# snu-mllab/Q-Palette

Hardware: AMD Instinct MI355X
Metric: decode tokens/s bs=1 Llama-3.1-8B @3.25b; achieved HBM GB/s vs peak (higher is better)
Workload: dtype f16 weights x f16 activations, f32 accumulate

## Files before the change

### include/qpal.h

```cpp
#ifndef QPAL_H
#define QPAL_H

#include <stdint.h>

#ifdef __cplusplus
extern "C" {
#endif

#define QPAL_VERSION 300

#define QPAL_OK 0
#define QPAL_E_SHAPE (-1)
#define QPAL_E_PARAM (-2)
#define QPAL_E_NULL (-3)
#define QPAL_E_ALIGN (-4)

#define QPAL_SPLIT_NONE 0
#define QPAL_SPLIT_ROWS 1
#define QPAL_SPLIT_COLS 2

int qpal_tcq_gemv(float *out, const void *c1, const void *c2, const void *x, const void *tlut,
                  int m, int n, int k, int S, int KV1, int KV2, int split, void *stream);

typedef struct qpal_tcq_job {
// ... 162 lines not shown

int qpal_lm_head_logits(const float *h_f32, long ld_h, const void *rms_w_f16, float rms_eps, const void *w_f16, float *logits_f32,
                        long ld_logits, int rows, int vocab, int k, void *stream);

int qpal_sample(const float *logits_f32, long ld_logits, int rows, int vocab, const float *temperature, const int *top_k,
                const float *top_p, const long *seed, const long *ctr, long *token, void *stream);

int qpal_token_logprob(const float *logits_f32, long ld_logits, int rows, int vocab, const long long *token, float *logprob,
                       float *lse, int *rank, const long long *active, void *stream);

int qpal_spec_draft(const int *hist, long ld_hist, const long *n_tok, const long *limit, const long *ext_draft, const int *ext_n,
                    int B, int K, int gmin, int gmax, int R, long max_len, long *tokens, int *seq, int *row0, long *pos0,
                    int *row_slot, long *row_ctr, int *n_draft, void *stream);
int qpal_spec_accept(const long *tokens, const long *drawn, const int *seq, const int *row0, int *hist, long ld_hist, long *n_tok,
                     long *limit, const long *eos, int B, int K, int R, long *out_tok, int *n_out, int *n_acc, void *stream);

int qpal_logit_process(const float *logits_f32, long ld_logits, float *out_f32, long ld_out, int rows, int vocab, const int *row_slot,
                       const long *ctr, int slots, const int *count, long ld_count, const float *repetition, const float *presence,
                       const float *frequency, const unsigned *mask, long ld_mask, const int *mask_on, const int *bias_id,
                       const float *bias_val, const int *bias_n, int bias_slots, const long *tokens, const int *row0, void *stream);
int qpal_logit_observe(int *count, long ld_count, int slots, int vocab, const int *slot, int slot0, const long *tokens,
                       const long *active, int n, void *stream);

#define QPAL_HESSIAN_TILE 128
int qpal_hessian_accum(double *H, double *colsum, const void *X_f16, long ld_x, int rows, int n, void *stream);

int qpal_lora_apply(float *out_f32, long ld_out, const void *in, int in_mode, float rms_eps, const void *rms_weight, const void *A,
                    const void *B, const int *blk_off, const int *blk_m, int P, const int *row_adapter, int rows, int k, int R, int N,
                    void *stream);

int qpal_plan_gemv(const int *rows, const int *steps1, const int *steps2, const int *flags, int njobs, int waves, int shared_staging,
                   int *out, int out_len);

int qpal_can_fuse_rotation(int n, int k);
int qpal_can_fuse_rotation_k(int n, int k, int K);

int qpal_calib_stream_read(const void *const *srcs, const long *bytes, int nseg, void *sink, int grid, void *stream);
int qpal_calib_decode_rate(const void *tlut, void *sink, int iters, int S, int KV, int grid, void *stream);

const char *qpal_error_string(int code);
int qpal_version(void);

#ifdef __cplusplus
}
#endif
#endif
```

### q-palette_amd/_native.py

```python
import ctypes
import os
import subprocess

_HERE = os.path.dirname(os.path.abspath(__file__))
SO_PATH = os.environ.get("QPAL_LIB") or os.path.join(_HERE, "libqpal_hip.so")
_lib = None

QPAL_SPLIT_NONE, QPAL_SPLIT_ROWS, QPAL_SPLIT_COLS = 0, 1, 2

_P, _I, _F = ctypes.c_void_p, ctypes.c_int, ctypes.c_float


class TcqJob(ctypes.Structure):
    _fields_ = [("out", _P), ("c1", _P), ("c2", _P), ("x", _P), ("tlut", _P), ("m", _I), ("k", _I),
                ("out_zeroed", _I), ("wscale", _P), ("oscale", _F), ("ldo", ctypes.c_long),
                ("x_had", _I), ("x_post", _F), ("x_su", _P), ("kv", _I),
                ("x_f32", _P),
                ("x_rms_eps", _F), ("x_rms_w", _P), ("accumulate", _I), ("kv2", _I), ("act_out", _P), ("x_hadk", _P), ("x_K", _I), ("act_su", _P)]


class LutJob(ctypes.Structure):
    _fields_ = [("out", _P), ("qweight", _P), ("x", _P), ("lut", _P), ("m", _I), ("k", _I), ("out_zeroed", _I),
                ("wscale", _P), ("oscale", _F), ("ldo", ctypes.c_long), ("x_had", _I), ("x_post", _F), ("x_su", _P),
                ("x_f32", _P),
                ("x_rms_eps", _F), ("x_rms_w", _P), ("accumulate", _I), ("act_out", _P), ("x_hadk", _P), ("x_K", _I), ("act_su", _P)]


PEER_WS_BYTES_PER_SLOT = 256
IPC_HANDLE_BYTES = 64


_SIGNATURES = {
    "qpal_tcq_gemv_multi": [ctypes.POINTER(TcqJob), _I, _I, _I, _I, _I, _I, _P, ctypes.c_long, _P],
    "qpal_lut_tc_gemv_multi": [ctypes.POINTER(LutJob), _I, _I, _I, _I, _P, ctypes.c_long, _P],
    "qpal_tcq_gemv": [_P, _P, _P, _P, _P, _I, _I, _I, _I, _I, _I, _I, _P],
    "qpal_tcq_dequant": [_P, _P, _P, _P, _I, _I, _I, _I, _I, _I, _P],
    "qpal_lut_tc_gemv": [_P, _P, _P, _P, _I, _I, _I, _I, _I, _P],
    "qpal_lut_tc_dequant": [_P, _P, _P, _I, _I, _I, _I, _P],
    "qpal_lut_simt_gemv": [_P, _P, _P, _P, _I, _I, _I, _I, _I, _P],
    "qpal_lut_simt_dequant": [_P, _P, _P, _I, _I, _I, _I, _P],
    "qpal_tc_to_simt": [_P, _P, _I, _I, _I, _I, _P],
    "qpal_plan_gemv": [ctypes.POINTER(_I), ctypes.POINTER(_I), ctypes.POINTER(_I), ctypes.POINTER(_I), _I, _I, _I, ctypes.POINTER(_I), _I],
    "qpal_can_fuse_rotation": [_I, _I],
    "qpal_can_fuse_rotation_k": [_I, _I, _I],
    "qpal_pack_tcq": [_P, _P, _I, _I, _I],
    "qpal_pack_tcq_states": [_P, _P, _I, _I, _I],
    "qpal_pack_lut_tc": [_P, _P, _I, _I, _I, _I],
    "qpal_pack_lut_simt": [_P, _P, _I, _I, _I, _I],
    "qpal_hadamard": [_P, _P, _P, _P, _P, _I, _I, _I, _I, _I, _I, _F, _P],
    "qpal_hadamard_rms": [_P, _P, _P, _F, _P, _P, _I, _I, _I, _F, _P],
    "qpal_hadamard_f32": [_P, _P, _P, _P, _I, _I, _I, _I, _F, _P],
    "qpal_rope_kv": [_P, _P, _P, _P, _P, _P, _P, _P, _I, _I, _I, ctypes.c_long, _P],
    "qpal_attn_decode": [_P, _P, _P, _P, _P, _I, _I, _I, ctypes.c_long, _F, _P],
    "qpal_attn_rope_decode": [_P, _P, _P, _P, _P, _P, _P, _P, _I, _I, _I, ctypes.c_long, _F, _P, ctypes.c_long, _P],
    "qpal_attn_ws_bytes": [_I, _I, _I, ctypes.c_long],
    "qpal_attn_rope_decode_batch": [_P, _P, _P, ctypes.c_long, _P, _P, _P, ctypes.c_long, _P, _P, _I, _I, _I, _I, ctypes.c_long, _F,
                                    _P, ctypes.c_long, _P],
    "qpal_attn_batch_ws_bytes": [_I, _I, _I, _I, ctypes.c_long],
    "qpal_attn_rope_prefill": [_P, _P, _P, ctypes.c_long, _P, _P, _P, ctypes.c_long, _P, _P, _I, _I, _I, _I, ctypes.c_long, _F,
                               _P, ctypes.c_long, _P],
    "qpal_attn_prefill_ws_bytes": [_I, _I, _I, _I, ctypes.c_long],
    "qpal_attn_rope_decode_batch_kv8": [_P, _P, _P, ctypes.c_long, _P, _P, _P, ctypes.c_long, _P, _P, _I, _I, _I, _I, ctypes.c_long,
                                        _F, _P, ctypes.c_long, _P],
    "qpal_attn_rope_prefill_kv8": [_P, _P, _P, ctypes.c_long, _P, _P, _P, ctypes.c_long, _P, _P, _I, _I, _I, _I, ctypes.c_long, _F,
                                   _P, ctypes.c_long, _P],
    "qpal_attn_rope_decode_batch_paged": [_P, _P, _P, ctypes.c_long, _P, _P, _P, ctypes.c_long, _P, _P, _P, ctypes.c_long, _I, _I, _I, _I,
                                          _I, _I, _I, _I, _F, _P, ctypes.c_long, _P],
    "qpal_attn_rope_prefill_paged": [_P, _P, _P, ctypes.c_long, _P, _P, _P, ctypes.c_long, _P, _P, _P, _I, _I, _I, _I,
                                     _I, _I, _I, _I, _F, _P, ctypes.c_long, _P],
    "qpal_attn_ragged_ws_bytes": [_I, _I, _I, _I, _I, ctypes.c_long],
    "qpal_attn_rope_prefill_ragged": [_P, _P, _P, ctypes.c_long, _P, _P, _P, ctypes.c_long, _P, _P, _P, _P, _I, _I, _I, _I, _I, _I, _I,
                                      ctypes.c_long, _F, _P, ctypes.c_long, _P],
    "qpal_attn_rope_prefill_ragged_paged": [_P, _P, _P, ctypes.c_long, _P, _P, _P, ctypes.c_long, _P, _P, _P, _P, _P, ctypes.c_long, _I,
                                            _I, _I, _I, _I, _I, _I, _I, _I, _I, _F, _P, ctypes.c_long, _P],
    "qpal_lm_head_argmax": [_P, _P, _F, _P, _P, _P, _P, ctypes.c_long, _I, _I, _P],
# ... 73 lines not shown
```

### q-palette_amd/csrc/qpal_capi.hip

```cpp
#include <stdio.h>
#include <hip/hip_runtime.h>
#include <math.h>
#include <stdlib.h>

#include "lut_kernels_api.h"
#include "tcq_kernels_api.h"
#include "tc_gemm16.h"
#include <string.h>

using namespace qpal;

namespace {

constexpr int kMaxBatch = 128;

int nbg_of(int n) { return n <= 8 ? 1 : n <= 16 ? 2 : n <= 32 ? 4 : n <= 64 ? 8 : n <= 80 ? 10 : 16; }
int waves_of(int nbg) { return gemv_waves<1>() == 8 ? 8 : (nbg >= 4 ? 8 : 16); }
int round_capacity(int waves) {
#if defined(QPAL_W8) && !defined(QPAL_W8_ONE)
    return waves == 8 ? 2 * kNumCU : kNumCU;
#else
    (void)waves;
    return kNumCU;
#endif
// ... 49 lines not shown
        if (!x_hadk || !p.x) return QPAL_E_NULL;
        if (x_f32 || x_rms_eps > 0.f) return QPAL_E_PARAM;
        if (!aligned(p.x, 16) || (x_su && !aligned(x_su, 16)) || !aligned(x_hadk, 2)) return QPAL_E_ALIGN;
        p.x_rot = kK28;
        p.x_hadk = static_cast<const uint16_t *>(x_hadk);
        p.x_su = static_cast<const uint16_t *>(x_su);
        p.x_pre = (float)(1.0 / sqrt((double)k));
        p.x_post = x_post;
        return QPAL_OK;
    }
    if (!rot_ok(n, k)) return QPAL_E_SHAPE;
    if (x_su && !aligned(x_su, 16)) return QPAL_E_ALIGN;
    if (x_f32) {
        p.x = static_cast<const uint16_t *>(x_f32);
        p.x_src_f32 = 1;
    }
    if (!p.x) return QPAL_E_NULL;
    if (x_rms_w && !aligned(x_rms_w, 16)) return QPAL_E_ALIGN;
    p.x_rms_eps = x_rms_eps > 0.f ? x_rms_eps : 0.f;
    p.x_rms_w = static_cast<const uint16_t *>(x_rms_w);
    if (!aligned(p.x, 16)) return QPAL_E_ALIGN;
    p.x_rot = k / 1024;
    p.x_su = static_cast<const uint16_t *>(x_su);
    p.x_pre = (float)(1.0 / sqrt((double)k));
    p.x_post = x_post;
    return QPAL_OK;
}

int nb_of(int n) { return n <= 1 ? 1 : n <= 2 ? 2 : n <= 4 ? 4 : 8; }

static int env_int(const char *name, int dflt) {
    const char *v = getenv(name);
    return v ? atoi(v) : dflt;
}

struct TapePlan {
    LaunchPlan lp;
    int cost;
    bool shared;
    bool ok;
};

TapePlan tape_plan(int lg_g, int rg, int st1, int st2, int W) {
    TapePlan tp{};
    const int G = 1 << lg_g, st = st1 + st2;
    tp.lp.lg_g = lg_g;
    tp.lp.rg = rg;
    const long T = (long)rg * st;
    if (st <= 0 || rg < 1 || rg > 255 || T < G) return tp;
    struct Piece { int row, stream, s0, len; };
    for (int m = 0; m < G; m++) {
        const long t0 = T * m / G, t1 = T * (m + 1) / G;
        Piece pc[kPlanWaves];
        int np = 0;
        for (int r = (int)(t0 / st); r < rg && (long)r * st < t1; r++)
            for (int sidx = 0; sidx < 2; sidx++) {
                const long seg0 = (long)r * st + (sidx ? st1 : 0), seg1 = seg0 + (sidx ? st2 : st1);
                const long a = seg0 > t0 ? seg0 : t0, b = seg1 < t1 ? seg1 : t1;
                if (b <= a) continue;
                if (np == W) return tp;
                pc[np++] = Piece{r, sidx, (int)(a - seg0), (int)(b - a)};
            }
        const long L = t1 - t0;
        struct Slot { int piece, part, ns; };
        Slot best_slots[kPlanWaves];
        int best_nslots = 0, best_cost = 1 << 30, best_long = 1 << 30;
// ... 6 lines not shown
                per[i] = pc[i].len / nw[i];
                if (per[i] < rowmin[pc[i].row]) rowmin[pc[i].row] = per[i];
            }
            for (int i = 1; i < np; i++)
                for (int k = i; k > 0; k--) {
                    const int x = order[k - 1], y = order[k];
                    const bool swap = rowmin[pc[y].row] != rowmin[pc[x].row] ? rowmin[pc[y].row] > rowmin[pc[x].row]
                                      : pc[y].row != pc[x].row             ? pc[y].row < pc[x].row
                                                                           : per[y] > per[x];
                    if (!swap) break;
                    order[k - 1] = y;
                    order[k] = x;
                }
            Slot slots[kPlanWaves];
            int simd[4] = {0, 0, 0, 0}, w = 0, longest = 0;
            for (int oi = 0; oi < np; oi++) {
                const int i = order[oi];
                for (int part = 0; part < nw[i]; part++, w++) {
                    const int ns = pc[i].len / nw[i] + (part < pc[i].len % nw[i] ? 1 : 0);
                    slots[w] = Slot{i, part, ns};
                    simd[w & 3] += ns;
                    if (ns > longest) longest = ns;
                }
            }
            int c = simd[0];
            for (int sd = 1; sd < 4; sd++) c = simd[sd] > c ? simd[sd] : c;
            if (c < best_cost || (c == best_cost && longest < best_long)) {
                best_cost = c;
                best_long = longest;
                best_nslots = w;
                for (int k = 0; k < w; k++) best_slots[k] = slots[k];
            }
        };
        for (int q = q0 > 0 ? q0 : 1; q <= 4 * q0 + 4; q++) {
            int nw[kPlanWaves], used = 0;
            for (int i = 0; i < np; i++) {
                nw[i] = (pc[i].len + q - 1) / q;
                used += nw[i];
            }
            if (used > W) continue;
            consider(nw);
            const int spare = W - used;
            if (spare == 0) continue;
            {
                int g[kPlanWaves];
                for (int i = 0; i < np; i++) g[i] = nw[i];
                for (int k = 0; k < spare; k++) {
                    int at = -1, worst = 0;
                    for (int i = 0; i < np; i++) {
                        const int pr = (pc[i].len + g[i] - 1) / g[i];
                        if (g[i] < pc[i].len && pr > worst) { worst = pr; at = i; }
                    }
                    if (at < 0) break;
                    g[at]++;
                }
                consider(g);
            }
            for (int t = 0; t < np; t++) {
                int g[kPlanWaves];
                for (int i = 0; i < np; i++) g[i] = nw[i];
                g[t] = g[t] + spare < pc[t].len ? g[t] + spare : pc[t].len;
                consider(g);
            }
        }
        if (best_cost == 1 << 30) return tp;
        int wave = best_nslots;
        for (int k = 0; k < best_nslots; k++) {
            const Piece &pp = pc[best_slots[k].piece];
            int nparts = 0;
            for (int k2 = 0; k2 < best_nslots; k2++) nparts += best_slots[k2].piece == best_slots[k].piece;
            const int base = pp.len / nparts, rem = pp.len % nparts, part = best_slots[k].part;
            const int s0 = pp.s0 + part * base + (part < rem ? part : rem);
            if (best_slots[k].ns > 0xffff || s0 > 0xffff) return tp;
            WaveEnt &e = tp.lp.w[m][k];
            e.a = (uint32_t)pp.row | ((uint32_t)pp.stream << 8) | (1u << 16);
            e.b = (uint32_t)s0 | ((uint32_t)best_slots[k].ns << 16);
// ... 8 lines not shown
        for (int sd = 0; sd < 4; sd++) {
            int c = 0;
            for (int q = 0; q < per; q++) c += (int)(tp.lp.w[m][sd + 4 * q].b >> 16);
            if (c > tp.cost) tp.cost = c;
        }
    }
    for (int r = 0; r < rg; r++) {
        int owners = 0;
        for (int m = 0; m < G; m++) {
            bool has = false;
            for (int w = 0; w < W; w++) has = has || ((tp.lp.w[m][w].a >> 16 & 1u) && (int)(tp.lp.w[m][w].a & 255u) == r);
            owners += has;
        }
        if (owners > 2) return tp;
        if (owners > 1) {
            tp.shared = true;
            for (int m = 0; m < G; m++)
                for (int w = 0; w < W; w++)
                    if ((tp.lp.w[m][w].a >> 16 & 1u) && (int)(tp.lp.w[m][w].a & 255u) == r) tp.lp.w[m][w].a |= 1u << 10;
        }
    }
    tp.ok = true;
    return tp;
}

int class_rows(const TcMultiParams &mp, int c, int rg) {
    int rows = 0;
    for (int j = 0; j < mp.njobs; j++)
        if (mp.job[j].cls == c) rows += (mp.job[j].nrows + rg - 1) / rg * rg;
    return rows;
}

void plan_launch(TcMultiParams &mp, const int *out_zeroed, int &grid, int waves = 16) {
    static const int force_g = env_int("QPAL_FORCE_G", 0);
    static const int force_rg = env_int("QPAL_FORCE_RG", 0);
    static const int share_on = env_int("QPAL_SHARE", env_int("QPAL_PAIR", 1));
    const int cap = round_capacity(waves);
    int ncls = 0, cst1[2] = {0, 0}, cst2[2] = {0, 0};
    for (int j = 0; j < mp.njobs; j++) {
        TcParams &p = mp.job[j];
        int c = 0;
        while (c < ncls && (cst1[c] != p.st1 || cst2[c] != p.st2)) c++;
        if (c == ncls) {
            if (ncls == 2) c = 1;
            else { cst1[c] = p.st1; cst2[c] = p.st2; ncls++; }
        }
        p.cls = c;
    }
    bool free_share = share_on != 0, swiglu = false;
    for (int j = 0; j < mp.njobs; j++) {
        const TcParams &p = mp.job[j];
        if (!((out_zeroed && out_zeroed[j]) || p.accumulate)) free_share = false;
        swiglu = swiglu || p.act_out != nullptr;
    }
    constexpr int kMemsetCost = 10;
    constexpr int kRoundCost = 4;
    struct Cand { TapePlan tp; int lg_g, rg; };
    static thread_local Cand cands[2][3 * 64];
    int ncand[2] = {0, 0};
    for (int c = 0; c < ncls; c++)
        for (int lg = 0; lg <= 2; lg++) {
            if (force_g > 0 && (1 << lg) != force_g) continue;
            if (swiglu && lg != 0) continue;
            for (int rg = 1; rg <= 16 << lg && rg <= 64; rg++) {
                if (force_rg > 0 && rg != force_rg) continue;
                if (swiglu && (rg & (rg - 1) || rg < 2 || rg > waves)) continue;
                TapePlan tp = tape_plan(lg, rg, cst1[c], cst2[c], waves);
                if (!tp.ok) continue;
                if (tp.shared && swiglu) continue;
                cands[c][ncand[c]++] = Cand{tp, lg, rg};
// ... 609 lines not shown
    if (grid > kNumCU) grid = kNumCU;
    return launch_simt_dequant(p, bits, vec, grid, static_cast<hipStream_t>(stream));
}

int qpal_tc_to_simt(void *dst_simt, const void *src_tc, int m, int k, int bits, int vec, void *stream) {
    if (!dst_simt || !src_tc) return QPAL_E_NULL;
    if (m <= 0 || k <= 0 || m % 32 || k % 32 || k % (32 * vec)) return QPAL_E_SHAPE;
    if (!(vec == 1 || vec == 2) || !lut_tc_ok(bits, vec) || ((long)bits * k) % (32 * vec)) return QPAL_E_PARAM;
    if (!aligned(dst_simt, 4) || !aligned(src_tc, 4)) return QPAL_E_ALIGN;
    hipStream_t s = static_cast<hipStream_t>(stream);
    hipError_t e = hipMemsetAsync(dst_simt, 0, (size_t)m * k / vec * bits / 8, s);
    if (e != hipSuccess) return (int)e;
    return launch_tc_to_simt(static_cast<uint32_t *>(dst_simt), static_cast<const uint32_t *>(src_tc), m, k, bits, vec, s);
}

int qpal_plan_gemv(const int *rows, const int *steps1, const int *steps2, const int *flags, int njobs, int waves, int shared_staging,
                   int *out, int out_len) {
    if (!rows || !steps1 || !steps2 || !flags || !out) return QPAL_E_NULL;
    if (njobs < 1 || njobs > kMaxJobs || (waves != 16 && waves != 8)) return QPAL_E_SHAPE;
    TcMultiParams mp{};
    mp.njobs = njobs;
    int zeroed[kMaxJobs] = {0};
    static const uint16_t dummy_x[8] = {0};
    for (int j = 0; j < njobs; j++) {
        TcParams &p = mp.job[j];
        p.nrows = rows[j];
        p.st1 = steps1[j];
        p.st2 = steps2[j];
        p.nsc1 = steps1[j] * 4;
        p.nsc2 = steps2[j] * 4;
        p.n = 1;
        p.k = (steps1[j] + steps2[j]) * 128;
        p.x = dummy_x;
        (void)shared_staging;
        zeroed[j] = flags[j] & 1;
        p.accumulate = (flags[j] >> 1) & 1;
        p.act_out = (flags[j] >> 2) & 1 ? reinterpret_cast<uint16_t *>(8) : nullptr;
        if (rows[j] < 1 || steps1[j] < 1 || steps2[j] < 0) return QPAL_E_SHAPE;
    }
    if (!gemv_classes_ok(mp)) return QPAL_E_PARAM;
    int grid = 0;
    plan_launch(mp, zeroed, grid, waves);
    const int need = 8 + 2 * (2 + 2 * kPlanMembers * kPlanWaves) + 4 * njobs;
    if (out_len < need) return QPAL_E_SHAPE;
    int o = 0;
    out[o++] = grid;
    out[o++] = mp.total_items;
    out[o++] = mp.ncls;
    out[o++] = mp.items0;
    out[o++] = 0;
    out[o++] = mp.cls_mask;
    out[o++] = kPlanMembers;
    out[o++] = kPlanWaves;
    for (int c = 0; c < 2; c++) {
        out[o++] = mp.plan[c].lg_g;
        out[o++] = mp.plan[c].rg;
        for (int m = 0; m < kPlanMembers; m++)
            for (int w = 0; w < kPlanWaves; w++) {
                out[o++] = (int)mp.plan[c].w[m][w].a;
                out[o++] = (int)mp.plan[c].w[m][w].b;
            }
    }
    for (int j = 0; j < njobs; j++) {
        out[o++] = mp.job[j].cls;
        out[o++] = mp.job[j].vrow0;
        out[o++] = mp.row_end[j];
        out[o++] = mp.job[j].sk;
    }
    return QPAL_OK;
}

int qpal_can_fuse_rotation(int n, int k) { return n >= 1 && k > 0 && rot_ok(n, k) ? 1 : 0; }
int qpal_can_fuse_rotation_k(int n, int k, int K) {
    if (K <= 1) return qpal_can_fuse_rotation(n, k);
    return rot_k28_ok(n, k, K, 64 * 1024) ? 1 : 0;
}

const char *qpal_error_string(int code) {
    switch (code) {
        case QPAL_OK: return "ok";
        case QPAL_E_SHAPE: return "unsupported shape (need m%32==0, k%32==0, 1<=n<=128; see include/qpal.h)";
        case QPAL_E_PARAM: return "unsupported quantizer parameters (S/KV/bits/vec/split)";
        case QPAL_E_NULL: return "null pointer";
        case QPAL_E_ALIGN: return "misaligned pointer";
        default: return code > 0 ? hipGetErrorString(static_cast<hipError_t>(code)) : "unknown qpal error";
    }
}

int qpal_version(void) { return QPAL_VERSION; }

}
```

### q-palette_amd/csrc/tc_kernels.h

```cpp
#pragma once
#include "qpal_common.h"
#include "wht64.h"
#include "rot_k28.h"

namespace qpal {

struct TcParams {
    float *out;
    uint16_t *wout;
    long ldo;
    long ldw;
    const uint32_t *c1;
    const uint32_t *c2;
    const uint16_t *x;
    const void *tab;
    int n;
    int k;
    int nrows;
    int nsc1, nsc2;
    int st1, st2;
    int col2;
    int sk;
    int nitems;
    int x_lds;
// ... 488 lines not shown
        xz = reinterpret_cast<const char *>(xs) + zero_off * 2;
        dead = (sv.nsc - (lane >> 4) + 3) >> 2;
        if (QPAL_ZERO_B != 0 && (c >> 1) >= n) dead = 0;
    }
    auto step_x = [&](int s, u32x4(&xb)[NBG][2]) {
        if constexpr (XLDS == 2 && NBG == 1) {
            const char *row = s < dead ? xl + s * 256 : xz;
            xb[0][0] = *reinterpret_cast<const u32x4 *>(row);
            xb[0][1] = *reinterpret_cast<const u32x4 *>(row + 16);
        } else {
            load_step_x<XLDS, NBG>(sv, xg, xs, k, n, zero_off, s, lane, xb);
        }
    };
    for (int s = s0; s < s1; s += 2) {
        {
            const int sn = s + 1 < s1 ? s + 1 : s;
            load_step_w_buf<Codec::NW>(rs, sn, lane, wb);
            __builtin_amdgcn_sched_barrier(0);
            u32x4 xb[NBG][2];
            step_x(s, xb);
            gemv_step_any<Codec, NBG>(lut, laneoff, w, xb, acc);
        }
        if (s + 1 < s1) {
            const int sn = s + 2 < s1 ? s + 2 : s + 1;
            load_step_w_buf<Codec::NW>(rs, sn, lane, w);
            __builtin_amdgcn_sched_barrier(0);
            u32x4 xb[NBG][2];
            step_x(s + 1, xb);
            gemv_step_any<Codec, NBG>(lut, laneoff, wb, xb, acc);
        }
    }
}

#ifdef QPAL_W8
template <int NBG>
constexpr int gemv_waves() { return 8; }
#define QPAL_GEMV_BOUNDS(NBG) __launch_bounds__(512, (NBG) <= 2 ? 4 : 2)
#else
template <int NBG>
constexpr int gemv_waves() { return NBG >= 4 ? 8 : 16; }
#define QPAL_GEMV_BOUNDS(NBG) __launch_bounds__(64 * gemv_waves<NBG>())
#endif
template <int NBG>
constexpr int scratch_bytes() { return NBG == 1 ? kScratchBytes : gemv_waves<NBG>() * 32 * 4 * 8 * NBG; }

template <int S>
struct TcqAny : TcqCodec<S, (S == 9 ? 8 : 10)> {
    static constexpr bool kAny = true;
    static constexpr int kMinKV = S == 9 ? 2 : S == 10 ? 8 : 9;
    static constexpr int kMaxKV = S == 9 ? 8 : 10;
};
template <class C>
constexpr bool is_any_v = requires { C::kAny; };

template <int S, class F>
__device__ __forceinline__ void dispatch_kv(int kv, F &&f) {
    static_for<TcqAny<S>::kMinKV, TcqAny<S>::kMaxKV + 1>([&](auto kc) {
        if (kv == decltype(kc)::value) f(kc);
    });
}

#ifdef QPAL_W8
constexpr int kEarlyXChunks = 1;
#else
constexpr int kEarlyXChunks = 2;
#endif
// ... 4 lines not shown
    int on;
    const uint16_t *su;
    const uint16_t *rw;
    float pre, post;
    int ie;
};

inline TcEarly early_args(const TcMultiParams &mp, int grid) {
    const TcParams &a = mp.job[0];
    TcEarly e{a.x, a.tab, a.n, a.k, a.x_lds && !a.x_rot && a.n <= 8 && a.n * a.k + 32 <= kEarlyXChunks * 64 * gemv_waves<1>() * 8 ? 1 : 0,
              a.x_su, a.x_rms_w, a.x_pre, a.x_post};
    if (a.x_lds && a.x_rot == kK28 && a.n == 1 && a.x_hadk && !a.x_src_f32 && !(a.x_rms_eps > 0.f)) {
        e.on = 2 | (kK28 << 4);
        e.rw = a.x_hadk;
    }
    if (a.x_lds && (a.x_rot == 2 || a.x_rot == 4) && a.n == 1) e.on = 2 | (a.x_src_f32 ? 4 : 0) | (a.x_rms_eps > 0.f ? 8 : 0) | (a.x_rot << 4);
    for (int j = 1; j < mp.njobs; j++) {
        const TcParams &b = mp.job[j];
        if (b.x != a.x || b.tab != a.tab || b.n != a.n || b.k != a.k || !b.x_lds || b.x_rot != a.x_rot || b.x_su != a.x_su ||
            b.x_rms_w != a.x_rms_w || b.x_src_f32 != a.x_src_f32 || (b.x_rms_eps > 0.f) != (a.x_rms_eps > 0.f) || b.x_hadk != a.x_hadk ||
            b.x_pre != a.x_pre || b.x_post != a.x_post)
            e.on = 0;
    }
    e.ie = 0;
    if (mp.ncls == 1 && mp.njobs <= 4 && mp.row_end[mp.njobs - 1] < 0x3ff && mp.plan[0].rg < 128) {
        e.ie = 1 << 30;
        for (int j = 0; j < 3; j++) e.ie |= (j < mp.njobs - 1 ? mp.row_end[j] : 0x3ff) << (10 * j);
        e.on |= (mp.plan[0].lg_g << 16) | (mp.plan[0].rg << 18);
    }
    if (grid >= mp.total_items) e.on |= 1 << 30;
    return e;
}

constexpr float kRmsPre = 0.015625f;
__device__ __forceinline__ void rot_stage1_regs(const u32x4 (&rq)[2][4], bool f32, bool rms, bool has_w, bool has_su, int wave, int lane,
                                                wht_float4 *d1buf, float *part) {
    float ss = 0.f;
    wht_half8 a[2];
#pragma unroll
    for (int kc = 0; kc < 2; kc++) {
        wht_half8 h;
        if (f32 || rms) {
            float f[8];
            if (f32) {
                const float4_t v0 = __builtin_bit_cast(float4_t, rq[kc][0]), v1 = __builtin_bit_cast(float4_t, rq[kc][1]);
#pragma unroll
                for (int e = 0; e < 4; e++) { f[e] = v0[e]; f[4 + e] = v1[e]; }
            } else {
                const wht_half8 hx = __builtin_bit_cast(wht_half8, rq[kc][0]);
#pragma unroll
                for (int e = 0; e < 8; e++) f[e] = (float)hx[e];
            }
            const wht_half8 wgt = __builtin_bit_cast(wht_half8, rq[kc][2]);
            const float pre = rms ? kRmsPre : 1.0f;
#pragma unroll
            for (int e = 0; e < 8; e++) {
                ss += f[e] * f[e];
                h[e] = (_Float16)(f[e] * pre * (has_w ? (float)wgt[e] : 1.0f));
            }
        } else {
            h = __builtin_bit_cast(wht_half8, rq[kc][0]);
        }
        if (has_su) h = h * __builtin_bit_cast(wht_half8, rq[kc][3]);
        a[kc] = h;
    }
    wht64_wg_stage1_pre(wave, lane, d1buf, a[0], a[1]);
    if (rms) {
        ss = wave_sum(ss);
        if (lane == 0) part[wave] = ss;
    }
}

template <class C1, class C2, int NBG, int ROT = 0>
__global__ QPAL_GEMV_BOUNDS(NBG) void tc_gemv_kernel(const uint16_t *ex, const void *etab, int en, int ek, int eon, int eie,
                                                       const uint16_t *esu, const uint16_t *erw, const TcMultiParams mp) {
    constexpr bool TWO = !std::is_void_v<C2>;
    using CB = std::conditional_t<TWO, C2, C1>;
    constexpr int W = gemv_waves<NBG>(), NT = 64 * W;
    static_assert(!ROT || NBG == 1, "fused rotation: batch 1 kernels");
    __shared__ __attribute__((aligned(16))) uint32_t lut[C1::LDS_DWORDS];
    __shared__ __attribute__((aligned(16))) unsigned char scratch[scratch_bytes<NBG>()];

    const int tid = threadIdx.x, lane = tid & 63;
    const int wave = __builtin_amdgcn_readfirstlane(tid >> 6);
    const uint32_t laneoff = (uint32_t)(lane & (C1::C - 1)) << 2;
#ifdef QPAL_STAMPS
    const unsigned long long t_entry = __builtin_amdgcn_s_memrealtime();
#endif

    const void *cur_tab = nullptr;
    const uint16_t *cur_x = nullptr;
    int cur_j = 0;
    constexpr int NV = (C1::CHUNKS + NT - 1) / NT;
    constexpr bool kXPerm = QPAL_XPERM_PLAIN != 0 && (ROT == 0 || ROT == 3);
    constexpr int kXL = kXPerm ? 2 : 1;
#ifndef QPAL_ANY_EARLY
#define QPAL_ANY_EARLY 1
#endif
    constexpr bool kEarly = NBG == 1 && (ROT == 0 || ROT == 3) && NV * NT <= 4096 && (QPAL_ANY_EARLY || !is_any_v<C1>);
    constexpr int EV = NV < 4 ? NV : 4;
    constexpr int XR = kEarlyXChunks;
    [[maybe_unused]] u32x4 exr[XR];
    [[maybe_unused]] uint32_t etv[EV][C1::RAWN];
    const bool early = kEarly && (eon & 1) != 0;
    constexpr int kRotTab = 6;
#ifndef QPAL_ROT_TAB_EARLY
#define QPAL_ROT_TAB_EARLY 1
#endif
    constexpr bool kRotTabEarly = QPAL_ROT_TAB_EARLY != 0;
    [[maybe_unused]] u32x4 rq_e[2][4];
    [[maybe_unused]] uint32_t rtv[kRotTab][C1::RAWN];
    constexpr bool kRotEarly = ROT == 1 && NBG == 1 && C1::CHUNKS <= kRotTab * (1024 - 64 * 4) && C1::NW + (TWO ? CB::NW : 0) <= 15;
    [[maybe_unused]] const bool rot_early = kRotEarly && (eon & 2) != 0;
    [[maybe_unused]] const int e_rot = (eon >> 4) & 63;
// ... 362 lines not shown
                cur_x = p.x;
            }
            if (p.tab != cur_tab) {
                C1::build(lut, p.tab, tid, NT);
                cur_tab = p.tab;
            }
            QPAL_STAMP(2);
            __syncthreads();
        }
        QPAL_STAMP(3);
        Acc<NBG> acc;
        static_for<0, NBG>([&](auto bc) {
            static_for<0, 4>([&](auto ac) {
                acc.v[decltype(bc)::value][decltype(ac)::value] = float4_t{0.f, 0.f, 0.f, 0.f};
            });
        });
        uint32_t wraw;
        asm volatile("" : "=v"(wraw));
        const int fr = lane & 31, fhi = lane >> 5;
        bool fin = ((ea >> 9) & 1u) != 0 && live && fhi == 0;
        if constexpr (ROT == 1) fin = ((ea >> 9) & 1u) != 0 && live && (fhi == 0 || (((ea >> 17) & 1u) != 0 && sr + 1 < nrows_j));
        const int fsrow = sr + fhi;
        if (p.wscale && fin) wraw = p.wscale[fsrow * 32 + fr];
        if constexpr (ANY) {
            dispatch_kv<C1::S_>(on2 ? kv2_j : kv1_j, [&](auto kc) {
                constexpr int KVr = decltype(kc)::value;
                using CK = TcqCodec<C1::S_, KVr>;
                auto &wk = reinterpret_cast<uint32_t(&)[KVr]>(w.a);
                const StreamView &sv = on2 ? sv2 : sv1;
                if (NBG == 1 && x_lds) gemv_run<CK, kXL, NBG>(wk, lut, laneoff, sv, rs_w, p.x, xs, p.k, p.n, zero_off, s0, s1, lane, acc);
                else gemv_run<CK, 0, NBG>(wk, lut, laneoff, sv, rs_w, p.x, xs, p.k, p.n, zero_off, s0, s1, lane, acc);
            });
        } else
        if constexpr (NBG == 1) {
            if (x_lds) {
                if constexpr (!TWO) gemv_run<C1, kXL, 1>(w.a, lut, laneoff, sv1, rs_w, p.x, xs, p.k, p.n, zero_off, s0, s1, lane, acc);
                else if (on2) gemv_run<CB, kXL, 1>(w.b, lut, laneoff, sv2, rs_w, p.x, xs, p.k, p.n, zero_off, s0, s1, lane, acc);
                else gemv_run<C1, kXL, 1>(w.a, lut, laneoff, sv1, rs_w, p.x, xs, p.k, p.n, zero_off, s0, s1, lane, acc);
            } else {
                if constexpr (!TWO) gemv_run<C1, 0, 1>(w.a, lut, laneoff, sv1, rs_w, p.x, xs, p.k, p.n, zero_off, s0, s1, lane, acc);
                else if (on2) gemv_run<CB, 0, 1>(w.b, lut, laneoff, sv2, rs_w, p.x, xs, p.k, p.n, zero_off, s0, s1, lane, acc);
                else gemv_run<C1, 0, 1>(w.a, lut, laneoff, sv1, rs_w, p.x, xs, p.k, p.n, zero_off, s0, s1, lane, acc);
            }
        } else {
            if constexpr (!TWO) gemv_run<C1, 0, NBG>(w.a, lut, laneoff, sv1, rs_w, p.x, xs, p.k, p.n, zero_off, s0, s1, lane, acc);
                else if (on2) gemv_run<CB, 0, NBG>(w.b, lut, laneoff, sv2, rs_w, p.x, xs, p.k, p.n, zero_off, s0, s1, lane, acc);
            else gemv_run<C1, 0, NBG>(w.a, lut, laneoff, sv1, rs_w, p.x, xs, p.k, p.n, zero_off, s0, s1, lane, acc);
        }
        QPAL_STAMP(4);

        {
            const int q = lane >> 4, cidx = lane & 15;
            static_for<0, NBG>([&](auto bc) {
                constexpr int grp = decltype(bc)::value;
                const int b = 8 * grp + (cidx >> 1);
                const bool writer = (cidx & 1) == 0 && b < p.n;
                float *dst = red + ((wave * p.n + (b < p.n ? b : 0)) * 32) + 2 * q;
                static_for<0, 4>([&](auto ac) {
                    constexpr int a = decltype(ac)::value;
                    const float4_t d = acc.v[grp][a];
                    const float v0 = d[0] + lane_xor<1>(d[1]);
                    const float v1 = d[2] + lane_xor<1>(d[3]);
                    if (writer) {
                        dst[8 * a] = v0;
                        dst[8 * a + 1] = v1;
                    }
// ... 171 lines not shown
```

### q-palette_amd/csrc/tcq_gemv.hip

```cpp
#include "tcq_launch.h"

namespace qpal {

int launch_tcq_gemv(const TcMultiParams &p, int S, int KV1, int KV2, int nbg, int grid, hipStream_t stream) {
    for (int j = 0; j < p.njobs; j++)
        if (p.job[j].x_rot) return nbg == 1 ? launch_tcq_gemv_rot(p, S, KV1, KV2, grid, stream) : QPAL_E_SHAPE;
#define QPAL_TCQ(S_, A_, B_)                                                                 \
    if (S == S_ && KV1 == A_ && KV2 == B_)                                                   \
        return nbg == 1 ? launch_one<S_, A_, B_, 1>(p, grid, stream) : nbg == 2 ? launch_one<S_, A_, B_, 2>(p, grid, stream) : \
               launch_tcq_gemv_wide(p, S, KV1, KV2, nbg, grid, stream);
#include "tcq_table.inc"
#undef QPAL_TCQ
    return QPAL_E_PARAM;
}

}
```

### q-palette_amd/csrc/tcq_kernels_api.h

```cpp
#pragma once
#include "tc_kernels.h"

namespace qpal {
int launch_tcq_gemv(const TcMultiParams &p, int S, int KV1, int KV2, int nbg, int grid, hipStream_t stream);
int launch_tcq_gemv_wide(const TcMultiParams &p, int S, int KV1, int KV2, int nbg, int grid, hipStream_t stream);
int launch_tcq_gemm_nbg1(const TcMultiParams &p, int S, int KV1, int KV2, int grid, hipStream_t stream);
int launch_tcq_gemm_nbg2(const TcMultiParams &p, int S, int KV1, int KV2, int grid, hipStream_t stream);
int launch_tcq_gemm_nbg4(const TcMultiParams &p, int S, int KV1, int KV2, int grid, hipStream_t stream);
int launch_tcq_gemm_nbg8(const TcMultiParams &p, int S, int KV1, int KV2, int grid, hipStream_t stream);
int launch_tcq_gemm_nbg10(const TcMultiParams &p, int S, int KV1, int KV2, int grid, hipStream_t stream);
int launch_tcq_gemm_nbg16(const TcMultiParams &p, int S, int KV1, int KV2, int grid, hipStream_t stream);
int launch_tcq_gemv_any(const TcMultiParams &p, int S, int grid, hipStream_t stream);
int launch_tcq_gemv_rot28(const TcMultiParams &p, int S, int KV1, int KV2, int grid, hipStream_t stream);
int launch_tcq_gemv_rot(const TcMultiParams &p, int S, int KV1, int KV2, int grid, hipStream_t stream);
int launch_tcq_dequant(const TcParams &p, int S, int KV1, int KV2, int grid, hipStream_t stream);
}
```

Before: 994.0.

## Add LDS weight ring with async buffer_load-to-LDS prefetch for batch-1 TCQ GEMV

Adds a ring-buffered GEMV path for batch-1 TCQ kernels. Each wave prefetches upcoming weight steps directly into LDS slots using buffer_load ... lds, with 2 or 3 slots in flight, then reads them back from LDS. The goal is to keep more HBM requests outstanding per wave so decode gets closer to bandwidth-bound streaming. The path is enabled by default when the codec has 6 to 8 dwords per lane, the longest piece is at least 3 steps and LDS fits. It also adds runtime planner knobs (min piece, grid cap), and it costs extra LDS, which can lower occupancy.

```diff
diff --git a/include/qpal.h b/include/qpal.h
--- a/include/qpal.h
+++ b/include/qpal.h
@@ -218,6 +218,9 @@
 int qpal_plan_gemv(const int *rows, const int *steps1, const int *steps2, const int *flags, int njobs, int waves, int shared_staging,
                    int *out, int out_len);
 
+int qpal_set_gemv_ring(int mode);
+int qpal_set_gemv_plan_knobs(int force_g, int force_rg, int min_piece, int grid_cap);
+
 int qpal_can_fuse_rotation(int n, int k);
 int qpal_can_fuse_rotation_k(int n, int k, int K);
 
diff --git a/q-palette_amd/_native.py b/q-palette_amd/_native.py
--- a/q-palette_amd/_native.py
+++ b/q-palette_amd/_native.py
@@ -41,6 +41,8 @@
     "qpal_lut_simt_dequant": [_P, _P, _P, _I, _I, _I, _I, _P],
     "qpal_tc_to_simt": [_P, _P, _I, _I, _I, _I, _P],
     "qpal_plan_gemv": [ctypes.POINTER(_I), ctypes.POINTER(_I), ctypes.POINTER(_I), ctypes.POINTER(_I), _I, _I, _I, ctypes.POINTER(_I), _I],
+    "qpal_set_gemv_ring": [_I],
+    "qpal_set_gemv_plan_knobs": [_I, _I, _I, _I],
     "qpal_can_fuse_rotation": [_I, _I],
     "qpal_can_fuse_rotation_k": [_I, _I, _I],
     "qpal_pack_tcq": [_P, _P, _I, _I, _I],
diff --git a/q-palette_amd/csrc/qpal_capi.hip b/q-palette_amd/csrc/qpal_capi.hip
--- a/q-palette_amd/csrc/qpal_capi.hip
+++ b/q-palette_amd/csrc/qpal_capi.hip
@@ -105,6 +105,14 @@
 static int env_int(const char *name, int dflt) {
     const char *v = getenv(name);
     return v ? atoi(v) : dflt;
+}
+
+struct PlanKnobs {
+    int force_g, force_rg, min_piece, grid_cap;
+};
+PlanKnobs &plan_knobs() {
+    static PlanKnobs k{env_int("QPAL_FORCE_G", 0), env_int("QPAL_FORCE_RG", 0), 0, 0};
+    return k;
 }
 
 struct TapePlan {
@@ -177,7 +185,8 @@
                 for (int k = 0; k < w; k++) best_slots[k] = slots[k];
             }
         };
-        for (int q = q0 > 0 ? q0 : 1; q <= 4 * q0 + 4; q++) {
+        const int min_piece = plan_knobs().min_piece;
+        for (int q = q0 > min_piece ? q0 : min_piece > 0 ? min_piece : 1; q <= 4 * q0 + 4 + min_piece; q++) {
             int nw[kPlanWaves], used = 0;
             for (int i = 0; i < np; i++) {
                 nw[i] = (pc[i].len + q - 1) / q;
@@ -186,7 +195,7 @@
             if (used > W) continue;
             consider(nw);
             const int spare = W - used;
-            if (spare == 0) continue;
+            if (spare == 0 || min_piece > 0) continue;
             {
                 int g[kPlanWaves];
                 for (int i = 0; i < np; i++) g[i] = nw[i];
@@ -261,10 +270,10 @@
 }
 
 void plan_launch(TcMultiParams &mp, const int *out_zeroed, int &grid, int waves = 16) {
-    static const int force_g = env_int("QPAL_FORCE_G", 0);
-    static const int force_rg = env_int("QPAL_FORCE_RG", 0);
+    const int force_g = plan_knobs().force_g, force_rg = plan_knobs().force_rg;
     static const int share_on = env_int("QPAL_SHARE", env_int("QPAL_PAIR", 1));
-    const int cap = round_capacity(waves);
+    int cap = round_capacity(waves);
+    if (plan_knobs().grid_cap > 0 && plan_knobs().grid_cap < cap) cap = plan_knobs().grid_cap;
     int ncls = 0, cst1[2] = {0, 0}, cst2[2] = {0, 0};
     for (int j = 0; j < mp.njobs; j++) {
         TcParams &p = mp.job[j];
@@ -940,7 +949,7 @@
         p.n = 1;
         p.k = (steps1[j] + steps2[j]) * 128;
         p.x = dummy_x;
-        (void)shared_staging;
+        p.x_lds = x_fits_lds(p.n, p.k);
         zeroed[j] = flags[j] & 1;
         p.accumulate = (flags[j] >> 1) & 1;
         p.act_out = (flags[j] >> 2) & 1 ? reinterpret_cast<uint16_t *>(8) : nullptr;
@@ -975,6 +984,24 @@
         out[o++] = mp.row_end[j];
         out[o++] = mp.job[j].sk;
     }
+    if (out_len >= need + 3) {
+        const int kv1 = (shared_staging >> 8) & 0xff, kv2 = (shared_staging >> 16) & 0xff;
+        int lds = 0, longest = 0;
+        const int depth = kv1 && waves == 16 ? gemv_ring_depth(mp, kv1, kv2, &lds, &longest) : (gemv_ring_depth(mp, 0, 0, &lds, &longest), 0);
+        out[o++] = depth;
+        out[o++] = lds;
+        out[o++] = longest;
+    }
+    return QPAL_OK;
+}
+
+int qpal_set_gemv_ring(int mode) {
+    gemv_ring_mode() = mode < -1 || mode > 3 ? -1 : mode;
+    return QPAL_OK;
+}
+int qpal_set_gemv_plan_knobs(int force_g, int force_rg, int min_piece, int grid_cap) {
+    plan_knobs() = PlanKnobs{force_g > 0 ? force_g : env_int("QPAL_FORCE_G", 0), force_rg > 0 ? force_rg : env_int("QPAL_FORCE_RG", 0),
+                             min_piece > 0 ? min_piece : 0, grid_cap > 0 ? grid_cap : 0};
     return QPAL_OK;
 }
 
diff --git a/q-palette_amd/csrc/tc_kernels.h b/q-palette_amd/csrc/tc_kernels.h
--- a/q-palette_amd/csrc/tc_kernels.h
+++ b/q-palette_amd/csrc/tc_kernels.h
@@ -544,6 +544,95 @@
     }
 }
 
+template <int NW>
+constexpr bool ring_codec_ok() { return NW >= 6 && NW <= 8; }
+template <int NW>
+constexpr int ring_na() { return NW >= 7 ? 4 : 3; }
+constexpr int kRingScratchBytes = 96 * 1024;
+constexpr int kRingSlot = 2048;
+constexpr int ring_offset(int waves, int n, int k) { return (waves * 32 * 4 * n + (n * k + 32) * 2 + 15) & ~15; }
+typedef uint32_t u32x3a __attribute__((ext_vector_type(3), aligned(16)));
+
+template <int ND>
+__device__ __forceinline__ void ring_fill_one(buf_rsrc_t rs, uint32_t voff, uint32_t lds) {
+    uint32_t keep;
+    if constexpr (ND == 4)
+        asm volatile("s_mov_b32 %0, m0\n\ts_mov_b32 m0, %3\n\ts_nop 0\n\tbuffer_load_dwordx4 %1, %2, 0 offen nt lds\n\ts_mov_b32 m0, %0"
+                     : "=&s"(keep) : "v"(voff), "s"(rs), "s"(lds) : "memory");
+    else
+        asm volatile("s_mov_b32 %0, m0\n\ts_mov_b32 m0, %3\n\ts_nop 0\n\tbuffer_load_dwordx3 %1, %2, 0 offen nt lds\n\ts_mov_b32 m0, %0"
+                     : "=&s"(keep) : "v"(voff), "s"(rs), "s"(lds) : "memory");
+}
+
+template <class Codec>
+__device__ __forceinline__ void gemv_run_ring(uint32_t (&w)[Codec::NW], const uint32_t *lut, uint32_t laneoff, const StreamView &sv,
+                                              buf_rsrc_t rs, const uint16_t *xs, int k, int n, int zero_off, int s0, int s1, int lane,
+                                              Acc<1> &acc, const unsigned char *slot0, uint32_t slot0_lds, int R) {
+    constexpr int NW = Codec::NW, NA = ring_na<NW>(), NB = NW - NA;
+    constexpr int SLOT = kRingSlot;
+    static_assert(ring_codec_ok<NW>(), "weight ring: 6..8 dwords per lane");
+    if (s0 >= s1) return;
+    const int c = lane & 15;
+    int b = c >> 1;
+    b = b < n ? b : n - 1;
+    const char *xl = reinterpret_cast<const char *>(xs) + (b * k + sv.col0 + (lane >> 4) * 32 + 16 * (c & 1)) * 2;
+    const char *xz = reinterpret_cast<const char *>(xs) + zero_off * 2;
+    int dead = (sv.nsc - (lane >> 4) + 3) >> 2;
+    if (QPAL_ZERO_B != 0 && (c >> 1) >= n) dead = 0;
+    auto step = [&](int s) {
+        const char *row = s < dead ? xl + s * 256 : xz;
+        u32x4 xb[1][2];
+        xb[0][0] = *reinterpret_cast<const u32x4 *>(row);
+        xb[0][1] = *reinterpret_cast<const u32x4 *>(row + 16);
+        gemv_step_any<Codec, 1>(lut, laneoff, w, xb, acc);
+    };
+    const uint32_t va = gemm_w_lane_off<NW>(lane);
+    const unsigned char *pa = slot0 + 16 * lane, *pb = pa + 1024;
+    auto fill = [&](int s, int slot) {
+        const uint32_t o = va + (uint32_t)s * gemm_w_step_bytes<NW>(), l = slot0_lds + (uint32_t)slot * SLOT;
+        ring_fill_one<NA>(rs, o, l);
+        ring_fill_one<NB>(rs, o + 4 * NA, l + 1024);
+    };
+#pragma unroll
+    for (int i = 0; i < NW; i++) asm volatile("" : "+v"(w[i]));
+    const int ns = s1 - s0;
+    if (ns > 1) fill(s0 + 1, 0);
+    if (ns > 2) fill(s0 + 2, 1);
+    if (R > 2 && ns > 3) fill(s0 + 3, 2);
+    step(s0);
+    int rd = 0;
+#pragma unroll 1
+    for (int s = s0 + 1; s < s1; s++) {
+        const int left = s1 - 1 - s, younger = left < R - 1 ? left : R - 1;
+        if (younger >= 2) asm volatile("s_waitcnt vmcnt(4)" ::: "memory");
+        else if (younger == 1) asm volatile("s_waitcnt vmcnt(2)" ::: "memory");
+        else asm volatile("s_waitcnt vmcnt(0)" ::: "memory");
+        {
+            const unsigned char *qa = pa + rd * SLOT, *qb = pb + rd * SLOT;
+            if constexpr (NA == 4) {
+                const u32x4 v = *reinterpret_cast<const u32x4 *>(qa);
+                w[0] = v.x; w[1] = v.y; w[2] = v.z; w[3] = v.w;
+            } else {
+                const u32x3a v = *reinterpret_cast<const u32x3a *>(qa);
+                w[0] = v[0]; w[1] = v[1]; w[2] = v[2];
+            }
+            if constexpr (NB == 4) {
+                const u32x4 v = *reinterpret_cast<const u32x4 *>(qb);
+                w[NA] = v.x; w[NA + 1] = v.y; w[NA + 2] = v.z; w[NA + 3] = v.w;
+            } else {
+                const u32x3a v = *reinterpret_cast<const u32x3a *>(qb);
+                w[NA] = v[0]; w[NA + 1] = v[1]; w[NA + 2] = v[2];
+            }
+        }
+        if (s + R < s1) {
+            asm volatile("s_waitcnt lgkmcnt(0)" ::: "memory");
+            fill(s + R, rd);
+        }
+        rd = rd + 1 == R ? 0 : rd + 1;
+        step(s);
+    }
+}
+
 #ifdef QPAL_W8
 template <int NBG>
 constexpr int gemv_waves() { return 8; }
@@ -614,6 +703,48 @@
     return e;
 }
 
+constexpr int kRingDepth = 2;
+inline int &gemv_ring_mode() {
+    static int mode = [] {
+        const char *v = getenv("QPAL_GEMV_RING");
+        return v ? atoi(v) : -1;
+    }();
+    return mode;
+}
+inline int gemv_ring_depth(const TcMultiParams &mp, int nw1, int nw2, int *lds_bytes = nullptr, int *longest_piece = nullptr) {
+    const int mode = gemv_ring_mode(), W = gemv_waves<1>();
+    int longest = 0;
+    for (int c = 0; c < mp.ncls && c < 2; c++)
+        for (int m = 0; m < (1 << mp.plan[c].lg_g) && m < kPlanMembers; m++)
+            for (int w = 0; w < W; w++)
+                if ((mp.plan[c].w[m][w].a >> 16) & 1u) longest = (int)(mp.plan[c].w[m][w].b >> 16) > longest ? (int)(mp.plan[c].w[m][w].b >> 16) : longest;
+    if (longest_piece) *longest_piece = longest;
+    if (lds_bytes) *lds_bytes = 0;
+#if defined(QPAL_STAMPS) || defined(QPAL_W8)
+    return 0;
+#endif
+    if (mode == 0 || W != 16) return 0;
+    if (nw1 < 6 || nw1 > 8 || (nw2 != 0 && (nw2 < 6 || nw2 > 8))) return 0;
+    if (mode < 0 && longest < 3) return 0;
+    int depth = mode == 2 ? 2 : mode == 3 ? 3 : kRingDepth;
+    for (; depth >= 2; depth--) {
+        bool fits = true;
+        int need = 0;
+        for (int j = 0; j < mp.njobs; j++) {
+            const TcParams &p = mp.job[j];
+            if (p.n < 1 || p.n > 8 || !p.x_lds || p.x_rot || p.dbg) return 0;
+            const int end = ring_offset(W, p.n, p.k) + W * depth * kRingSlot;
+            fits = fits && end <= kRingScratchBytes;
+            need = end > need ? end : need;
+        }
+        if (fits) {
+            if (lds_bytes) *lds_bytes = 64 * 1024 + need;
+            return depth;
+        }
+    }
+    return 0;
+}
+
 constexpr float kRmsPre = 0.015625f;
 __device__ __forceinline__ void rot_stage1_regs(const u32x4 (&rq)[2][4], bool f32, bool rms, bool has_w, bool has_su, int wave, int lane,
                                                 wht_float4 *d1buf, float *part) {
@@ -653,15 +784,16 @@
     }
 }
 
-template <class C1, class C2, int NBG, int ROT = 0>
+template <class C1, class C2, int NBG, int ROT = 0, int RING = 0>
 __global__ QPAL_GEMV_BOUNDS(NBG) void tc_gemv_kernel(const uint16_t *ex, const void *etab, int en, int ek, int eon, int eie,
                                                        const uint16_t *esu, const uint16_t *erw, const TcMultiParams mp) {
     constexpr bool TWO = !std::is_void_v<C2>;
     using CB = std::conditional_t<TWO, C2, C1>;
     constexpr int W = gemv_waves<NBG>(), NT = 64 * W;
     static_assert(!ROT || NBG == 1, "fused rotation: batch 1 kernels");
+    static_assert(!RING || (NBG == 1 && ROT == 0 && !is_any_v<C1> && C1::LDS_DWORDS * 4 == 64 * 1024), "weight ring: plain batch-1 TCQ kernels");
     __shared__ __attribute__((aligned(16))) uint32_t lut[C1::LDS_DWORDS];
-    __shared__ __attribute__((aligned(16))) unsigned char scratch[scratch_bytes<NBG>()];
+    __shared__ __attribute__((aligned(16))) unsigned char scratch[RING ? kRingScratchBytes : scratch_bytes<NBG>()];
 
     const int tid = threadIdx.x, lane = tid & 63;
     const int wave = __builtin_amdgcn_readfirstlane(tid >> 6);
@@ -1090,6 +1222,15 @@
                 else gemv_run<CK, 0, NBG>(wk, lut, laneoff, sv, rs_w, p.x, xs, p.k, p.n, zero_off, s0, s1, lane, acc);
             });
         } else
+        if constexpr (RING != 0) {
+            const int R = (eon >> 26) & 3;
+            const unsigned char *slot0 = scratch + ring_offset(W, p.n, p.k) + wave * R * kRingSlot;
+            const uint32_t slot0_lds = __builtin_amdgcn_readfirstlane(
+                (uint32_t)(uintptr_t)(const __attribute__((address_space(3))) unsigned char *)slot0);
+            if constexpr (!TWO) gemv_run_ring<C1>(w.a, lut, laneoff, sv1, rs_w, xs, p.k, p.n, zero_off, s0, s1, lane, acc, slot0, slot0_lds, R);
+            else if (on2) gemv_run_ring<CB>(w.b, lut, laneoff, sv2, rs_w, xs, p.k, p.n, zero_off, s0, s1, lane, acc, slot0, slot0_lds, R);
+            else gemv_run_ring<C1>(w.a, lut, laneoff, sv1, rs_w, xs, p.k, p.n, zero_off, s0, s1, lane, acc, slot0, slot0_lds, R);
+        } else
         if constexpr (NBG == 1) {
             if (x_lds) {
                 if constexpr (!TWO) gemv_run<C1, kXL, 1>(w.a, lut, laneoff, sv1, rs_w, p.x, xs, p.k, p.n, zero_off, s0, s1, lane, acc);
diff --git a/q-palette_amd/csrc/tcq_gemv.hip b/q-palette_amd/csrc/tcq_gemv.hip
--- a/q-palette_amd/csrc/tcq_gemv.hip
+++ b/q-palette_amd/csrc/tcq_gemv.hip
@@ -5,6 +5,10 @@
 int launch_tcq_gemv(const TcMultiParams &p, int S, int KV1, int KV2, int nbg, int grid, hipStream_t stream) {
     for (int j = 0; j < p.njobs; j++)
         if (p.job[j].x_rot) return nbg == 1 ? launch_tcq_gemv_rot(p, S, KV1, KV2, grid, stream) : QPAL_E_SHAPE;
+    if (nbg == 1) {
+        const int depth = gemv_ring_depth(p, KV1, KV2);
+        if (depth) return launch_tcq_gemv_ring(p, S, KV1, KV2, depth, grid, stream);
+    }
 #define QPAL_TCQ(S_, A_, B_)                                                                 \
     if (S == S_ && KV1 == A_ && KV2 == B_)                                                   \
         return nbg == 1 ? launch_one<S_, A_, B_, 1>(p, grid, stream) : nbg == 2 ? launch_one<S_, A_, B_, 2>(p, grid, stream) : \
diff --git a/q-palette_amd/csrc/tcq_gemv_ring.hip b/q-palette_amd/csrc/tcq_gemv_ring.hip
--- /dev/null
+++ b/q-palette_amd/csrc/tcq_gemv_ring.hip
@@ -0,0 +1,24 @@
+#include "tcq_kernels_api.h"
+
+namespace qpal {
+
+template <int S, int KV1, int KV2>
+static int launch_ring(const TcMultiParams &mp, int depth, int grid, hipStream_t stream) {
+    TcEarly e = early_args(mp, grid);
+    e.on |= depth << 26;
+    using C1 = TcqCodec<S, KV1>;
+    using C2 = std::conditional_t<KV2 == 0, void, TcqCodec<S, KV2 == 0 ? KV1 : KV2>>;
+    hipLaunchKernelGGL((tc_gemv_kernel<C1, C2, 1, 0, 1>), dim3(grid), dim3(64 * gemv_waves<1>()), 0, stream, e.x, e.tab, e.n, e.k, e.on, e.ie, e.su, e.rw, mp);
+    return (int)hipGetLastError();
+}
+
+int launch_tcq_gemv_ring(const TcMultiParams &p, int S, int KV1, int KV2, int depth, int grid, hipStream_t stream) {
+    if (depth < 2 || depth > 3) return QPAL_E_PARAM;
+#define QPAL_RING(S_, A_, B_) \
+    if (S == S_ && KV1 == A_ && KV2 == B_) return launch_ring<S_, A_, B_>(p, depth, grid, stream);
+    QPAL_RING(9, 6, 0) QPAL_RING(9, 7, 0) QPAL_RING(9, 8, 0) QPAL_RING(9, 6, 7) QPAL_RING(9, 7, 8) QPAL_RING(10, 8, 0)
+#undef QPAL_RING
+    return QPAL_E_PARAM;
+}
+
+}
diff --git a/q-palette_amd/csrc/tcq_kernels_api.h b/q-palette_amd/csrc/tcq_kernels_api.h
--- a/q-palette_amd/csrc/tcq_kernels_api.h
+++ b/q-palette_amd/csrc/tcq_kernels_api.h
@@ -3,6 +3,7 @@
 
 namespace qpal {
 int launch_tcq_gemv(const TcMultiParams &p, int S, int KV1, int KV2, int nbg, int grid, hipStream_t stream);
+int launch_tcq_gemv_ring(const TcMultiParams &p, int S, int KV1, int KV2, int depth, int grid, hipStream_t stream);
 int launch_tcq_gemv_wide(const TcMultiParams &p, int S, int KV1, int KV2, int nbg, int grid, hipStream_t stream);
 int launch_tcq_gemm_nbg1(const TcMultiParams &p, int S, int KV1, int KV2, int grid, hipStream_t stream);
 int launch_tcq_gemm_nbg2(const TcMultiParams &p, int S, int KV1, int KV2, int grid, hipStream_t stream);
```

Result: slower. 924.0 (-7.0%).
